# jianhao2016/AllSet

Measured on AMD Instinct MI355X. Metric: edges*d aggregated / sec (V->E->V layer fwd+bwd), higher is better.
Workload: dtype f32

## Files before the change

allset_amd/_lib.py:

```python
from __future__ import annotations

import ctypes
import os
from ctypes import c_char_p, c_float, c_int, c_int64, c_size_t, c_uint64, c_void_p, POINTER

import torch

LIB_PATH = os.path.join(os.path.dirname(os.path.abspath(__file__)), "liballset_hip.so")
ABI_VERSION = 15
CORE_ABI_VERSION = 1

SUM, MEAN, MAX, MIN = 0, 1, 2, 3
F32, BF16 = 0, 1
REDUCE_AS_TREE = 0x100
ARITH_AUTO, ARITH_BF16X6, ARITH_FP16X3 = 0, 1, 2
ACT_NONE, ACT_RELU, ACT_ELU = 0, 1, 2
REDUCE_CODES = {"add": SUM, "sum": SUM, "mean": MEAN, "max": MAX, "min": MIN}

_P = c_void_p
SIGNATURES = {
    "allset_version": [],
    "allset_core_version": [],
    "allset_csr_build_workspace_bytes": [c_int64, c_int64, POINTER(c_size_t)],
    "allset_csr_build": [_P, _P, c_int64, c_int64, c_int64, c_int64, _P, _P, _P, _P, c_size_t, _P],
    "allset_segreduce_fwd": [c_int, c_int, _P, _P, _P, _P, c_int64, _P, c_int64, _P, c_int64, c_int64, c_int64, _P],
    "allset_segreduce_fwd_ex": [c_int, c_int, c_int, c_int64, _P, _P, _P, _P, _P, c_int64, _P, c_int64, _P, c_int64, c_int64,
                                c_int64, _P],
    "allset_segmax_bwd": [_P, _P, _P, _P, _P, _P, c_int64, _P, c_int64, c_int64, c_int64, c_int64, _P],
    "allset_sddmm_rowdot": [c_int, _P, _P, _P, c_int64, _P, c_int64, _P, _P, c_int64, c_int64, c_int64, _P],
    "allset_pma_fwd": [c_int, _P, _P, _P, _P, c_int64, c_float, _P, c_int64, _P, _P, c_int64, c_int64, c_int64, c_int64, _P],
    "allset_pma_fwd_ex": [c_int, c_int, c_int64, _P, _P, _P, _P, _P, c_int64, c_float, _P, c_int64, _P, _P, c_int64, c_int64,
                          c_int64, c_int64, _P],
    "allset_pma_fwd_ld": [c_int, c_int, c_int64, _P, _P, _P, _P, c_int64, _P, c_int64, c_float, _P, c_int64, _P, _P, c_int64,
                          c_int64, c_int64, c_int64, _P],
    "allset_pma_bwd_stats_ld": [c_int, _P, c_int64, _P, c_int64, _P, _P, _P, c_int64, c_int64, c_int64, c_int64, _P],
    "allset_pma_bwd_src_ld": [c_int, c_int, c_int64, _P, _P, _P, _P, _P, c_int64, _P, c_int64, _P, c_int64, c_float, _P, c_int64,
                              _P, c_int64, c_int64, c_int64, c_int64, _P],
    "allset_pma_attention": [_P, _P, _P, _P, _P, c_float, _P, c_int64, c_int64, _P],
    "allset_pma_bwd_stats": [c_int, _P, c_int64, _P, c_int64, _P, _P, _P, c_int64, c_int64, c_int64, _P],
    "allset_pma_bwd_src": [c_int, _P, _P, _P, _P, c_int64, _P, c_int64, _P, c_float, _P, c_int64, _P,
                           c_int64, c_int64, c_int64, c_int64, _P],
    "allset_pma_bwd_src_ex": [c_int, c_int, c_int64, _P, _P, _P, _P, _P, c_int64, _P, c_int64, _P, c_float, _P, c_int64, _P,
                              c_int64, c_int64, c_int64, c_int64, _P],
    "allset_ln_fwd": [_P, c_int64, _P, _P, c_float, c_int, c_float, c_uint64, _P, c_int64, _P, c_int64, c_int64, _P, _P],
    "allset_ln_bwd_partials": [c_int64, c_int64, POINTER(c_int64)],
    "allset_ln_bwd": [_P, c_int64, _P, c_int64, _P, _P, c_int, c_float, c_uint64, _P, c_int64, _P, c_int64,
                      c_int64, c_int64, _P, _P],
# ... 206 lines not shown
    "allset_han_block_relabel": [_P, _P, _P, c_int64, c_int64, _P, _P, _P, _P, _P],
    "allset_han_block_compact_fixed": [_P, _P, _P, _P, _P, _P, _P, _P, c_int64, c_int64, _P, _P, _P, _P, _P],
    "allset_han_block_transpose": [_P, _P, _P, c_int64, c_int64, _P, _P, _P, _P],
    "allset_han_block_compact": [_P, _P, _P, _P, _P, _P, c_int64, c_int64, c_int64, c_int64, _P, _P, _P],
    "allset_han_block_hop_fwd": [c_int64, _P, _P, _P, _P, _P, c_int64, c_float, _P, c_float, c_uint64, _P, _P, c_int64, _P, c_int64, _P,
                                 _P, c_int64, c_int64, c_int64, c_int64, _P],
    "allset_han_block_hop_bwd_stats": [_P, c_int64, _P, _P, c_int64, _P, c_int64, _P, _P, c_float, _P, c_int64, _P, _P, c_int64, c_int64,
                                       c_int64, _P],
    "allset_han_block_hop_bwd_src": [c_int64, _P, _P, _P, _P, _P, _P, c_int64, _P, c_int64, _P, c_float, c_float, c_uint64, _P, _P,
                                     c_int64, _P, c_int64, c_int64, c_int64, c_int64, _P],
    "allset_hattn_supported": [],
    "allset_hattn_coef": [c_int64, _P, _P, _P, _P, _P, _P, c_float, c_float, c_uint64, _P, _P, _P, _P, _P, c_int64, c_int64, c_int64, _P],
    "allset_hattn_hop": [c_int64, _P, _P, _P, _P, _P, _P, _P, c_int64, _P, c_int, c_float, c_uint64, _P, c_int, _P, c_int64, c_int64,
                         c_int64, c_int64, c_int64, _P],
    "allset_hattn_bwd_vertex": [c_int64, _P, _P, _P, _P, _P, _P, _P, _P, c_float, _P, c_int64, _P, c_int64, _P, c_int64, _P, c_int64, _P,
                                _P, _P, c_int64, _P, _P, _P, c_int64, c_int64, c_int64, c_int64, _P],
    "allset_hattn_bwd_edge": [c_int64, _P, _P, _P, c_int64, c_int64, _P],
    "allset_spgemm_bool_bins": [POINTER(c_int64)],
    "allset_spgemm_bool_workspace_bytes": [c_int64, POINTER(c_size_t)],
    "allset_spgemm_bool_count": [_P, _P, _P, _P, c_int64, c_int64, c_int64, _P, _P, c_size_t, _P],
    "allset_spgemm_bool_fill": [_P, _P, _P, _P, c_int64, c_int64, c_int64, _P, c_int64, _P, _P, c_size_t, _P],
    "allset_loo_supported": [c_int64],
    "allset_loo_long_threshold": [],
    "allset_loo_rows": [_P, _P, _P, c_int64, _P, _P, _P, c_int64, _P, c_int64, c_int64, c_int64, c_int64, c_int64, _P],
    "allset_loo_softmax_supported": [c_int64, c_int64],
    "allset_loo_softmax_fwd": [_P, _P, _P, _P, c_int64, c_float, _P, c_int64, _P, _P, c_int64, c_int64, c_int64, c_int64, c_int64,
                               c_int64, _P],
    "allset_loo_softmax_bwd": [_P, _P, _P, _P, c_int64, c_float, _P, c_int64, _P, _P, c_int64, _P, _P, c_int64, _P, _P, _P, c_int64,
                               c_int64, c_int64, c_int64, c_int64, c_int64, _P],
    "allset_scan_rows_supported": [c_int64],
    "allset_scan_rows": [_P, _P, _P, c_int64, _P, _P, c_int64, _P, c_int64, c_int, c_int64, c_int64, c_int64, c_int64, _P],
    "allset_scan_collect": [_P, _P, _P, c_int64, _P, _P, c_int64, _P, _P, c_int, c_float, c_uint64, _P, _P, c_int64, c_int64, c_int64,
                            c_int64, c_int64, _P],
}
EXPORTED_SYMBOLS = sorted(list(SIGNATURES) + ["allset_last_error"])


class AllSetHipError(RuntimeError):
    pass


_lib = None


def load() -> ctypes.CDLL:
    global _lib
    if _lib is not None:
        return _lib
    if not os.path.exists(LIB_PATH):
        raise AllSetHipError(
            f"{LIB_PATH} not found: build it with `python -m allset_amd.build` "
            "(allset_amd has no CPU / eager fallback for the aggregation path)")
    lib = ctypes.CDLL(LIB_PATH)
    for name, argtypes in SIGNATURES.items():
        fn = getattr(lib, name)
        fn.argtypes = argtypes
        fn.restype = c_int
    lib.allset_fused_linear_mask_words.restype = c_int64
    lib.allset_gemm_x6_plane_bytes.restype = c_int64
    lib.allset_gemm_f16x3_plane_bytes.restype = c_int64
    lib.allset_gemm_x6_lnb_partials.restype = c_int64
    lib.allset_input_linear_k.restype = c_int64
    lib.allset_linear_bf16_mask_pitch.restype = c_int64
    lib.allset_sparse_linear_pitch.restype = c_int64
    lib.allset_last_error.argtypes = []
    lib.allset_last_error.restype = c_char_p
# ... 53 lines not shown
```

allset_amd/csrc/segreduce.hip:

```cpp
#include "common.h"
#include "flat_rows.h"
#include "mfma.h"

namespace allset {

enum { kModeSum = 0, kModeExt = 1 };
constexpr int kUnroll = 8;
#ifndef ALLSET_SEG_UNROLL_ONE_SLOT
#define ALLSET_SEG_UNROLL_ONE_SLOT 8
#endif
#ifndef ALLSET_SEG_MAX_LPR
#define ALLSET_SEG_MAX_LPR 64
#endif
constexpr int kBwdUnroll = 4;

template <typename T, int VEC, int LPR, int MODE, bool WEIGHTED>
__global__ __launch_bounds__(kBlock) void segreduce_kernel(
    const int32_t* __restrict__ rowptr, const int32_t* __restrict__ col, const float* __restrict__ w,
    const T* __restrict__ x, int64_t ldx, T* __restrict__ out, int64_t ldo,
    int32_t* __restrict__ argext, int n_t, int d, int mean, float sign, const int32_t* __restrict__ row_order) {
  constexpr int NS = kWave / LPR;
  constexpr int U = NS == 1 ? ALLSET_SEG_UNROLL_ONE_SLOT : kUnroll;
  const unsigned blk = xcd_contiguous_block(blockIdx.x, gridDim.x);
  const int slot_row = static_cast<int>(blk) * kWavesPerBlock + (threadIdx.x >> 6);
// ... 263 lines not shown
  for (int k = 0; k < VEC; ++k) { g.v[k] = 0.f; ap[k] = -1; }
  if (active) {
    g = load_vec<float, VEC>(gout + static_cast<int64_t>(row) * ldg + c0);
    if constexpr (MODE == kModeExt) load_vec_i32<VEC>(argext + static_cast<int64_t>(row) * d + c0, ap);
  }
  for (int base = start; base < end; base += kWave) {
    const int n = min(kWave, end - base);
    const int my_col = lane < n ? col[base + lane] : 0;
    for (int j = 0; j < n; j += NS * kUnroll) {
      Raw<float, VEC> raw[kUnroll];
#pragma unroll
      for (int u = 0; u < kUnroll; ++u) {
        const int jj = j + u * NS + slot;
        const int src = __shfl(my_col, jj & (kWave - 1));
        if (jj < n && active) raw[u] = load_raw<float, VEC>(x + static_cast<int64_t>(src) * ldx + c0);
        else raw[u] = zero_raw<float, VEC>();
      }
      float res = 0.f;
#pragma unroll
      for (int u = 0; u < kUnroll; ++u) {
        const FVec<VEC> v = unpack<float, VEC>(raw[u]);
        float part = 0.f;
#pragma unroll
        for (int k = 0; k < VEC; ++k) {
          if constexpr (MODE == kModeExt) part = (ap[k] == base + j + u * NS + slot) ? fmaf(v.v[k], g.v[k], part) : part;
          else part = fmaf(v.v[k], g.v[k], part);
        }
        part = slot_sum<LPR>(part);
        res = (li == u) ? part : res;
      }
      const int jo = j + li * NS + slot;
      if (li < kUnroll && jo < n) gw[base + jo] = res * scale;
    }
  }
}


template <typename T, int VEC, int LPR>
static void launch_segreduce(int mode_ext, bool weighted, unsigned grid, hipStream_t st,
                             const int32_t* rowptr, const int32_t* col, const float* w, const T* x,
                             int64_t ldx, T* out, int64_t ldo, int32_t* argext, int n_t, int d, int mean,
                             float sign, const int32_t* row_order) {
  if (!mode_ext) {
    if (weighted) segreduce_kernel<T, VEC, LPR, kModeSum, true><<<grid, kBlock, 0, st>>>(rowptr, col, w, x, ldx, out, ldo, argext, n_t, d, mean, sign, row_order);
    else          segreduce_kernel<T, VEC, LPR, kModeSum, false><<<grid, kBlock, 0, st>>>(rowptr, col, w, x, ldx, out, ldo, argext, n_t, d, mean, sign, row_order);
  } else {
    if (weighted) segreduce_kernel<T, VEC, LPR, kModeExt, true><<<grid, kBlock, 0, st>>>(rowptr, col, w, x, ldx, out, ldo, argext, n_t, d, mean, sign, row_order);
    else          segreduce_kernel<T, VEC, LPR, kModeExt, false><<<grid, kBlock, 0, st>>>(rowptr, col, w, x, ldx, out, ldo, argext, n_t, d, mean, sign, row_order);
  }
}

template <typename T, int WIDE>
static void dispatch_flat(bool weighted, hipStream_t st, const int32_t* rowptr, const int32_t* col, const float* w,
                          const T* x, int64_t ldx, T* out, int64_t ldo, int n_t, int d, int mean) {
  with_lpr(pick_lpr(d, WIDE), [&](auto lpr) {
    const unsigned grid = flat_grid<lpr()>(n_t);
    if (weighted) segreduce_flat_kernel<T, WIDE, lpr(), true><<<grid, kBlock, 0, st>>>(rowptr, col, w, x, ldx, out, ldo, n_t, d, mean);
    else          segreduce_flat_kernel<T, WIDE, lpr(), false><<<grid, kBlock, 0, st>>>(rowptr, col, w, x, ldx, out, ldo, n_t, d, mean);
  });
}

template <typename T, int WIDE>
static void dispatch_segreduce(bool wide_ok, int mode_ext, bool weighted, unsigned grid, hipStream_t st,
                               const int32_t* rowptr, const int32_t* col, const float* w, const T* x, int64_t ldx,
                               T* out, int64_t ldo, int32_t* argext, int n_t, int d, int mean, float sign,
                               const int32_t* row_order) {
// ... 102 lines not shown
}

extern "C" int allset_sddmm_rowdot(int reduce, const int32_t* rowptr, const int32_t* col, const float* x,
                                   int64_t ldx, const float* gout, int64_t ldg, const int32_t* argext,
                                   float* gw, int64_t n_t, int64_t n_s, int64_t d, void* stream) {
  clear_error();
  ALLSET_REQUIRE(reduce >= ALLSET_SUM && reduce <= ALLSET_MIN, "sddmm_rowdot: bad reduce %d", reduce);
  ALLSET_REQUIRE(n_t >= 0 && n_s >= 0 && d >= 0, "sddmm_rowdot: negative size");
  ALLSET_REQUIRE(n_t < INT32_MAX && n_s < INT32_MAX && d < INT32_MAX, "sddmm_rowdot: size exceeds int32");
  if (n_t == 0 || n_s == 0) return ALLSET_OK;
  ALLSET_REQUIRE(rowptr && col && x && gout && gw, "sddmm_rowdot: null pointer");
  ALLSET_REQUIRE(ldx >= d && ldg >= d, "sddmm_rowdot: leading dimension smaller than d");
  const bool ext = (reduce == ALLSET_MAX || reduce == ALLSET_MIN);
  ALLSET_REQUIRE(!ext || argext, "sddmm_rowdot: MAX/MIN need argext");
  const hipStream_t st = static_cast<hipStream_t>(stream);
  const unsigned grid = row_grid(n_t);
  const int mean = (reduce == ALLSET_MEAN);
  const int nt = static_cast<int>(n_t), di = static_cast<int>(d);
  const bool vec4 = (d % 4 == 0) && d <= 256 && (ldx % 4 == 0) && (ldg % 4 == 0) && aligned16(x) && aligned16(gout) &&
                    (!ext || aligned16(argext));
  if (vec4) {
    with_lpr(pick_lpr(d), [&](auto lpr) {
      if (ext) sddmm_rowdot_vec_kernel<lpr(), kModeExt><<<grid, kBlock, 0, st>>>(rowptr, col, x, ldx, gout, ldg, argext, gw, nt, di, mean);
      else     sddmm_rowdot_vec_kernel<lpr(), kModeSum><<<grid, kBlock, 0, st>>>(rowptr, col, x, ldx, gout, ldg, nullptr, gw, nt, di, mean);
    });
  } else if (ext) {
    sddmm_rowdot_kernel<kModeExt><<<grid, kBlock, 0, st>>>(rowptr, col, x, ldx, gout, ldg, argext, gw, nt, di, mean);
  } else {
    sddmm_rowdot_kernel<kModeSum><<<grid, kBlock, 0, st>>>(rowptr, col, x, ldx, gout, ldg, nullptr, gw, nt, di, mean);
  }
  ALLSET_LAUNCH_CHECK();
  return ALLSET_OK;
}
```

allset_amd/dist.py:

```python
from __future__ import annotations

import os
from typing import Callable, Optional, Tuple

import torch
import torch.distributed as dist
import torch.nn.functional as F

Tensor = torch.Tensor



def vertex_block(n_v: int, world: int, rank: int) -> Tuple[int, int, int]:
    per = (n_v + world - 1) // world
    return rank * per, (rank + 1) * per, per * world


def partition_hyperedges(sizes: Tensor, world: int, method: str = "contiguous") -> Tensor:
    sizes = sizes.to(torch.int64)
    n_e = sizes.numel()
    if method == "contiguous":
        csum = torch.cumsum(sizes, 0)
        total = int(csum[-1]) if n_e else 0
        mid = csum - sizes // 2
# ... 361 lines not shown
    @staticmethod
    def forward(ctx, part, hg, is_min):
        halo = hg.halo
        r = halo.rank
        v = -part if is_min else part
        key = (_ordered_key(v) << 8) | (255 - r)
        if halo.world == 1 or _skip_collective(halo.group):
            recv = key
        else:
            recv = _all_to_all_rows(key.contiguous(), halo.need_counts, halo.send_counts, halo.group)
        best = torch.full((halo.block, key.shape[1]), -1, dtype=torch.int64, device=key.device)
        if recv.shape[0]:
            best = best.scatter_reduce(0, halo.send_idx.view(-1, 1).expand_as(recv), recv, "amax", include_self=True)
        best_c = best.index_select(0, halo.send_idx)
        if not (halo.world == 1 or _skip_collective(halo.group)):
            best_c = _all_to_all_rows(best_c, halo.send_counts, halo.need_counts, halo.group)
        won = best_c == key
        any_inc = best >= 0
        bits = (best >> 8) & 0xFFFFFFFF
        bits = torch.where(bits >= 0x80000000, bits - 0x80000000, 0xFFFFFFFF - bits)
        val = torch.where(bits >= 0x80000000, bits - 0x100000000, bits).to(torch.int32).view(torch.float32)
        out = torch.where(any_inc, -val if is_min else val, torch.zeros_like(val))
        ctx.save_for_backward(won)
        ctx.halo = halo
        return out

    @staticmethod
    def backward(ctx, gout):
        (won,) = ctx.saved_tensors
        g_c = ctx.halo._gather(gout.contiguous())
        return torch.where(won, g_c, torch.zeros_like(g_c)), None, None


def _hip_deepsets(x, inc, norm, aggr):
    from . import functional as AF
    return AF.deepsets_aggregate(x, inc, norm, aggr)


class HipPmaKernels:

    @staticmethod
    def aggregate(V, alpha, inc, heads, slope):
        from . import functional as AF
        return AF.pma_aggregate(V, alpha, inc, heads, slope)[0]

    @staticmethod
    def fwd(V, alpha, inc, heads, slope):
        from . import ops
        from .functional import _variant, _sizes
        csr = inc.by_dst
        return ops.pma_fwd(csr.rowptr, csr.col, alpha, V, heads, slope, inc.n_dst,
                           variant=_variant(csr, "pma_fwd", inc.n_dst, V, heads), row_order=csr.row_order, sizes=_sizes(csr, V, heads))

    @staticmethod
    def bwd_stats(out, gout, m, l):
        from . import ops
        return ops.pma_bwd_stats(out, gout, m, l)

    @staticmethod
    def merge_pack(o_loc, m_loc, l_loc, m_glob, heads):
        from . import ops
        return ops.pma_merge_pack(o_loc, m_loc, l_loc, m_glob, heads)

    @staticmethod
    def bwd_src(inc, alpha, V, gout, stats, slope):
        from . import ops
        from .functional import _variant, _sizes
        T = inc.by_src
        return ops.pma_bwd_src(T.rowptr, T.col, alpha, V, gout, stats, slope,
                               variant=_variant(T, "pma_bwd_src", V.shape[0], V, alpha.shape[1]), row_order=T.row_order,
                               sizes=_sizes(T, V, alpha.shape[1]))


def _bn_scope(valid_rows: int, group):
    from . import dense
    return dense.sync_bn_rows(valid_rows, group)


def _valid_rows(lo: int, hi: int, n: int) -> int:
    return max(0, min(int(hi), int(n)) - int(lo))


def sharded_deepsets_layer(v2e_conv, e2v_conv, x_owned: Tensor, hg: ShardedHypergraph, aggr: str = "add",
                           dropout: float = 0.0, training: bool = False, group=None,
                           aggregate: Callable = _hip_deepsets, norm: Optional[Tensor] = None,
                           dropout_out: Optional[float] = None) -> Tensor:
    if aggr not in ("add", "sum", "mean", "max", "min"):
        raise ValueError(f"aggr {aggr!r}")
    vv = _valid_rows(hg.v_lo, hg.v_hi, hg.n_v)
    norm = hg.norm if norm is None else norm
    p_out = dropout if dropout_out is None else dropout_out
    use_halo = hg.halo is not None and hg.halo_v2e is not None
    with _bn_scope(vv, group):
        h = v2e_conv._mlp_act(v2e_conv.f_enc, x_owned, v2e_conv.dropout)
    if use_halo:
        e = aggregate(halo_gather(h, hg.halo), hg.halo_v2e, norm, aggr)
    else:
        h_full = all_gather_rows(h, group)
        e = aggregate(h_full, hg.v2e, norm, aggr)
    with _bn_scope(e.shape[0], group):
        e = v2e_conv._mlp_act(v2e_conv.f_dec, e, dropout)
        g = e2v_conv._mlp_act(e2v_conv.f_enc, e, e2v_conv.dropout)
    if aggr in ("max", "min") and use_halo:
        v = _HaloExtremeMerge.apply(aggregate(g, hg.halo_e2v, norm, aggr), hg, aggr == "min")
    elif aggr in ("max", "min"):
        partial = aggregate(g, hg.e2v, norm, aggr)
        v = _ShardedExtremeMerge.apply(partial, hg.local_vertex_has_incidence(), hg, group, aggr == "min")
    elif use_halo:
        v = halo_scatter_add(aggregate(g, hg.halo_e2v, norm, "add"), hg.halo)
    else:
        partial = aggregate(g, hg.e2v, norm, "add")
        v = reduce_scatter_rows(partial, group)
    if aggr == "mean":
        v = v / hg.owned_vertex_degree(group).clamp(min=1).view(-1, 1)
    with _bn_scope(vv, group):
        return e2v_conv._mlp_act(e2v_conv.f_dec, v, p_out)


class _ShardedPmaE2V(torch.autograd.Function):

    @staticmethod
    def forward(ctx, V, alpha, hg, heads, slope, group, K, use_halo=False):
        halo = hg.halo if use_halo else None
        inc = hg.halo_e2v if halo is not None else hg.e2v
        in_dtype = V.dtype
        alpha = alpha.float()
        o_loc, m_loc, l_loc = K.fwd(V, alpha, inc, heads, slope)
        o_loc = o_loc.float()
        n, d = o_loc.shape
        C = d // heads
        has = l_loc > 0
        neg_inf = torch.full_like(m_loc, float("-inf"))
        m_eff = torch.where(has, m_loc, neg_inf)
        if halo is not None:
            m_owned = halo._scatter_max(m_loc.contiguous())
            m_gc = halo.gather_narrow(m_owned)
            if hasattr(K, "merge_pack"):
                packed = K.merge_pack(o_loc, m_loc, l_loc, m_gc, heads)
            else:
                w = l_loc * torch.exp(m_loc - m_gc)
                packed = torch.cat([(o_loc.view(n, heads, C) * w.unsqueeze(-1)).view(n, d), w], dim=1)
            red = halo.scatter_add_narrow(packed)
            numer, l_g = red[:, :d], red[:, d:].contiguous()
            inv = torch.where(l_g > 0, 1.0 / (l_g + 1e-16), torch.zeros_like(l_g))
# ... 725 lines not shown
```

allset_amd/functional.py:

```python
from __future__ import annotations

from typing import Optional, Tuple

import torch
from torch.autograd.function import once_differentiable

from . import _lib, ops
from ._lib import MAX, MEAN, MIN, REDUCE_CODES, SUM
from .incidence import Incidence, LeaveOneOutIncidence

Tensor = torch.Tensor


def _variant(csr, kind: str, n_rows: int, x: Tensor, heads: int = 1) -> int:
    es = x.element_size()
    wide = 16 // es
    d = x.shape[1]
    ok = (d % wide == 0 and d <= 64 * wide and x.stride(0) % wide == 0 and x.data_ptr() % 16 == 0
          and (d // max(heads, 1)) % wide == 0)
    if not ok:
        return 1
    if d * es <= 128 and csr.max_deg <= 512:
        return 2
    return csr.variant(kind, n_rows)
# ... 24 lines not shown
def _check_rows(x: Tensor, inc: Incidence) -> None:
    if not (inc.src_extent <= x.shape[0] <= inc.n_src):
        raise ValueError(f"source matrix has {x.shape[0]} rows; incidence needs between {inc.src_extent} "
                         f"and {inc.n_src}")


class _RouteWeights(torch.autograd.Function):

    @staticmethod
    def forward(ctx, w, perm, inv_perm):
        ctx.save_for_backward(inv_perm)
        return w.index_select(0, perm)

    @staticmethod
    @once_differentiable
    def backward(ctx, g):
        (inv_perm,) = ctx.saved_tensors
        return g.index_select(0, inv_perm), None, None


def _routed(norm: Tensor, inc: Incidence, dst: bool) -> Tensor:
    csr = inc.by_dst if dst else inc.by_src
    perm, inv = (inc.perm_dst_long(), inc.inv_perm_dst()) if dst else (inc.perm_src_long(), inc.inv_perm_src())
    if norm.grad_fn is None:
        return _RouteWeights.apply(norm.reshape(-1).to(torch.float32), perm, inv)
    cache = norm.__dict__.setdefault("_allset_routed", {})
    key = (id(csr), norm._version, torch.is_grad_enabled())
    hit = cache.get(key)
    if hit is None:
        hit = cache[key] = _RouteWeights.apply(norm.reshape(-1).to(torch.float32), perm, inv)
    return hit


class _SegReduce(torch.autograd.Function):
    @staticmethod
    def forward(ctx, x: Tensor, w_dst: Optional[Tensor], w_src: Optional[Tensor], inc: Incidence, reduce: int):
        csr = inc.by_dst
        ext = reduce in (MAX, MIN)
        out, arg = ops.segreduce(reduce, csr.rowptr, csr.col, w_dst, x, inc.n_dst, want_arg=ext,
                                 variant=1 if ext else _variant(csr, "segreduce", inc.n_dst, x), row_order=csr.row_order,
                                 split=_split(csr, x))
        need_gw = w_dst is not None and ctx.needs_input_grad[1]
        ctx.inc, ctx.reduce, ctx.n_s, ctx.need_gw = inc, reduce, x.shape[0], need_gw
        ctx.save_for_backward(x if need_gw else None, w_dst, w_src, arg)
        return out

    @staticmethod
    @once_differentiable
    def backward(ctx, gout: Tensor):
        x, w_dst, w_src, arg = ctx.saved_tensors
        inc, reduce = ctx.inc, ctx.reduce
        T = inc.by_src
        gx = gw = None
        gout = gout.contiguous()
        if reduce in (MAX, MIN) or ctx.need_gw:
            if gout.dtype != torch.float32:
                raise _lib.AllSetHipError("max/min backward and weight gradients are fp32-only; bf16 storage covers "
                                          "sum/mean and the PMA path")
        if ctx.needs_input_grad[0]:
            if w_dst is not None and w_src is None:
                w_src = w_dst[inc.pos_dst_of_src().long()]
            if reduce in (SUM, MEAN):
                if reduce == MEAN:
                    inv = inc.inv_count_by_src()
                    w_src = inv if w_src is None else w_src * inv
                gx, _ = ops.segreduce(SUM, T.rowptr, T.col, w_src, gout, ctx.n_s,
                                      variant=_variant(T, "segreduce", ctx.n_s, gout), row_order=T.row_order,
                                      split=_split(T, gout) if ctx.n_s == T.n_rows else -1)
            else:
                gx = ops.segmax_bwd(T.rowptr, T.col, inc.pos_dst_of_src(), w_src, arg, gout, ctx.n_s)
        if ctx.need_gw:
            csr = inc.by_dst
            gw = ops.sddmm_rowdot(reduce, csr.rowptr, csr.col, x, gout, arg)
        return gx, gw, None, None, None


def deepsets_aggregate(x: Tensor, inc: Incidence, norm: Optional[Tensor] = None, aggr: str = "add") -> Tensor:
    if aggr not in REDUCE_CODES:
        raise ValueError(f"unknown aggr {aggr!r}")
    _lib.require_device(x)
    _check_rows(x, inc)
    if norm is not None and norm.requires_grad:
        w_dst = _routed(norm, inc, True)
        w_src = _routed(norm, inc, False).detach()
    else:
        w_dst, w_src = inc.weights(norm)
    return _SegReduce.apply(x, w_dst, w_src, inc, REDUCE_CODES[aggr])


def _loo_expand(x: Tensor, loo: LeaveOneOutIncidence, s_src: Optional[Tensor], s_seg: Optional[Tensor]) -> Tensor:
    return ops.loo_rows(loo.e_rowptr, loo.e_col, x, s_src, s_seg, long_seg=loo.long_seg if loo.n_long else None, n_long=loo.n_long)


def _loo_collect(y: Tensor, loo: LeaveOneOutIncidence, s_seg: Optional[Tensor], w_inc: Optional[Tensor], n_rows: int) -> Tensor:
    t = ops.loo_rows(loo.e_rowptr, None, y, None, s_seg, long_seg=loo.long_seg if loo.n_long else None, n_long=loo.n_long)
    out, _ = ops.segreduce(SUM, loo.v_rowptr, loo.v_col, w_inc, t, n_rows)
    return out


class _LooV2E(torch.autograd.Function):
    @staticmethod
    def forward(ctx, x: Tensor, loo: LeaveOneOutIncidence, f):
        ctx.loo, ctx.f, ctx.n_rows = loo, f, x.shape[0]
        return _loo_expand(x, loo, f.v2e_src, f.v2e_seg)

    @staticmethod
    @once_differentiable
    def backward(ctx, gout: Tensor):
        f = ctx.f
        return _loo_collect(gout.contiguous(), ctx.loo, f.v2e_seg, f.v2e_src_inc, ctx.n_rows), None, None


class _LooE2V(torch.autograd.Function):
    @staticmethod
    def forward(ctx, y: Tensor, loo: LeaveOneOutIncidence, f):
        ctx.loo, ctx.f = loo, f
        return _loo_collect(y, loo, f.e2v_seg, f.e2v_row_inc, loo.n_dst)

    @staticmethod
    @once_differentiable
# ... 912 lines not shown
```

allset_amd/layers.py:

```python
from __future__ import annotations

import math
from typing import Tuple, Optional, Union

import os

import torch
import torch.nn as nn
import torch.nn.functional as F

from . import dense
from . import functional as AF
from .incidence import Incidence, LooDirection, cached_incidence

Tensor = torch.Tensor
EdgeIndex = Union[Tensor, Incidence]


def glorot(tensor: Optional[Tensor]) -> None:
    if tensor is not None:
        bound = math.sqrt(6.0 / (tensor.size(-2) + tensor.size(-1)))
        with torch.no_grad():
            tensor.uniform_(-bound, bound)

# ... 432 lines not shown
    def __repr__(self):
        return '{}({}, {}, heads={})'.format(self.__class__.__name__, self.in_channels, self.out_channels, self.heads)


class HalfNLHconv(nn.Module):

    def __init__(self, in_dim, hid_dim, out_dim, num_layers, dropout, Normalization='bn', InputNorm=False,
                 heads=1, attention=True):
        super().__init__()
        self.attention = attention
        self.dropout = dropout
        if self.attention:
            self.prop = PMA(in_dim, hid_dim, out_dim, num_layers, heads=heads)
        elif num_layers > 0:
            self.f_enc = MLP(in_dim, hid_dim, hid_dim, num_layers, dropout, Normalization, InputNorm)
            self.f_dec = MLP(hid_dim, hid_dim, out_dim, num_layers, dropout, Normalization, InputNorm)
        else:
            self.f_enc = nn.Identity()
            self.f_dec = nn.Identity()

    def reset_parameters(self):
        if self.attention:
            self.prop.reset_parameters()
        else:
            for f in (self.f_enc, self.f_dec):
                if not isinstance(f, nn.Identity):
                    f.reset_parameters()

    def takes_pre_dropout(self, x: Tensor) -> bool:
        if self.attention:
            return self.prop.takes_pre_dropout(x)
        return isinstance(self.f_enc, MLP) and self.f_enc.takes_pre_dropout(x)

    def forward(self, x, edge_index: EdgeIndex, norm, aggr='add', _post_dropout: Optional[float] = None, _pre_dropout: float = 0.0):
        post = _post_dropout is not None
        if _pre_dropout and not (self.takes_pre_dropout(x) and (aggr is not None or self.attention)):
            raise ValueError("HalfNLHconv.forward(_pre_dropout=...) needs takes_pre_dropout(x)")
        if isinstance(edge_index, LooDirection):
            if self.attention:
                if not edge_index.attention:
                    raise NotImplementedError("exclude-self data without the expansion reaches the PMA conv (attention=True, "
                                              "AllSetTransformer) only when asked for: preprocessing.exclude_self(data, normtype, "
                                              "attention=True) takes the leave-one-out softmax; or expand the edge list with "
                                              "preprocessing.expand_edge_index instead")
                if norm is not None and norm.requires_grad:
                    raise NotImplementedError("exclude-self data without the expansion takes no per-incidence weight (LearnMask is a "
                                              "parameter per EXPANDED incidence); expand the edge list with "
                                              "preprocessing.expand_edge_index instead")
                if post and self.training:
                    return self.prop.forward_exclude_self(x, edge_index, _post=float(_post_dropout), _pre=float(_pre_dropout))
                x = self.prop.forward_exclude_self(x, edge_index, _pre=float(_pre_dropout))
                return relu_dropout(x, _post_dropout, self.training) if post else x
            if norm is not None and norm.requires_grad:
                raise NotImplementedError("exclude-self data without the expansion takes no per-incidence weight (LearnMask is a parameter "
                                          "per EXPANDED incidence); expand the edge list with preprocessing.expand_edge_index instead")
            if aggr is None:
                raise ValueError("aggr was not passed!")
            x = self._mlp_act(self.f_enc, x, self.dropout, pre=_pre_dropout)
            x = AF.deepsets_aggregate_exclude_self(x, edge_index.loo, edge_index.direction, aggr, edge_index.normtype)
            return self._mlp_act(self.f_dec, x, _post_dropout if post else 0.0)
        if self.attention:
            if post and self.training:
                return self.prop(x, edge_index, _post=float(_post_dropout), _pre=float(_pre_dropout))
            x = self.prop(x, edge_index, _pre=float(_pre_dropout))
            return relu_dropout(x, _post_dropout, self.training) if post else x
        if aggr is None:
            raise ValueError("aggr was not passed!")
        x = self._mlp_act(self.f_enc, x, self.dropout, pre=_pre_dropout)
        inc = _as_incidence(edge_index, x.shape[0])
        x = AF.deepsets_aggregate(x, inc, norm, aggr)
        return self._mlp_act(self.f_dec, x, _post_dropout if post else 0.0)

    def _mlp_act(self, mlp, x, p, in_cb: int = 0, out_cb: int = 0, pre: float = 0.0):
        if isinstance(mlp, MLP):
            return mlp(x, _post=p, _in_cb=in_cb, _out_cb=out_cb, _pre=pre)
        return relu_dropout(mlp(x), p, self.training)
```

allset_amd/ops.py:

```python
from __future__ import annotations

from collections import defaultdict
from ctypes import byref, c_int64 as c_int64_t, c_size_t, c_void_p
from typing import Dict, List, NamedTuple, Optional, Sequence, Tuple

import torch

from . import _lib
from ._lib import check, ptr, require_device, stream_of, on_device

Tensor = torch.Tensor


class KernelTimer:

    def __init__(self):
        self.events: Dict[str, List[Tuple[torch.cuda.Event, torch.cuda.Event, int]]] = defaultdict(list)

    def summary(self) -> Dict[str, Dict[str, float]]:
        out = {}
        for name, evs in self.events.items():
            ms = [s.elapsed_time(e) for s, e, _ in evs]
            out[name] = dict(calls=len(ms), total_ms=sum(ms), avg_ms=sum(ms) / len(ms),
                             algo_bytes=sum(b for _, _, b in evs) / len(evs))
# ... 185 lines not shown
    return order.to(torch.int32).contiguous()


def segreduce(reduce: int, rowptr: Tensor, col: Tensor, w: Optional[Tensor], x: Tensor, n_t: int,
              want_arg: bool = False, variant: int = 0, row_order: Optional[Tensor] = None, split: int = -1
              ) -> Tuple[Tensor, Optional[Tensor]]:
    dev = require_device(rowptr, col, w, x)
    code = _dtype_code(x, "segreduce")
    es = x.element_size()
    x = _rowmajor(x)
    n_s, d = x.shape
    out = torch.empty((n_t, d), dtype=x.dtype, device=dev)
    arg = torch.empty((n_t, d), dtype=torch.int32, device=dev) if want_arg else None
    if w is not None:
        _f32(w, "segreduce weights")
        w = w.contiguous()
    nnz = col.numel()
    algo = nnz * (es * d + 4 + (4 if w is not None else 0)) + (n_t + 1) * 4 + n_t * d * es
    with on_device(dev), _timed("segreduce_fwd", dev, algo):
        if row_order is not None and row_order.numel() != n_t:
            row_order = None
        lib = _lib.load()
        if 0 < split < n_t and not want_arg and rowptr.numel() == n_t + 1:
            check(lib.allset_segreduce_fwd_ex(reduce, code, 1, nnz, None, ptr(rowptr), ptr(col), ptr(w), ptr(x), _ld(x),
                                              ptr(out), max(d, 1), None, split, n_s, d, stream_of(dev)), "allset_segreduce_fwd_ex")
            check(lib.allset_segreduce_fwd_ex(reduce, code, 2, nnz, None, ptr(rowptr[split:]), ptr(col), ptr(w), ptr(x), _ld(x),
                                              ptr(out[split:]), max(d, 1), None, n_t - split, n_s, d, stream_of(dev)),
                  "allset_segreduce_fwd_ex")
        else:
            check(lib.allset_segreduce_fwd_ex(reduce, code, variant, nnz, ptr(row_order), ptr(rowptr), ptr(col), ptr(w), ptr(x), _ld(x),
                                              ptr(out), max(d, 1), ptr(arg), n_t, n_s, d, stream_of(dev)),
                  "allset_segreduce_fwd_ex")
    return out, arg


def segmax_bwd(rowptrT: Tensor, colT: Tensor, posT: Tensor, wT: Optional[Tensor], argext: Tensor, gout: Tensor,
               n_s: int) -> Tensor:
    dev = require_device(rowptrT, colT, posT, wT, argext, gout)
    _f32(gout, "segmax_bwd")
    gout = _rowmajor(gout)
    n_t, d = gout.shape
    if colT.numel() == 0:
        return torch.zeros((n_s, d), dtype=gout.dtype, device=dev)
    gx = torch.empty((n_s, d), dtype=gout.dtype, device=dev)
    algo = colT.numel() * (4 * d + 4 * d + 8) + (n_s + 1) * 4 + n_s * d * 4
    with on_device(dev), _timed("segmax_bwd", dev, algo):
        check(_lib.load().allset_segmax_bwd(ptr(rowptrT), ptr(colT), ptr(posT), ptr(wT), ptr(argext), ptr(gout),
                                            _ld(gout), ptr(gx), max(d, 1), n_s, n_t, d, stream_of(dev)),
              "allset_segmax_bwd")
    return gx


def sddmm_rowdot(reduce: int, rowptr: Tensor, col: Tensor, x: Tensor, gout: Tensor, argext: Optional[Tensor]) -> Tensor:
    dev = require_device(rowptr, col, x, gout, argext)
    _f32(x, "sddmm_rowdot")
    x, gout = _rowmajor(x), _rowmajor(gout)
    n_s, d = x.shape
    n_t = gout.shape[0]
    gw = torch.empty(col.numel(), dtype=torch.float32, device=dev)
    if col.numel() == 0:
        return gw
    algo = col.numel() * (4 * d + 8) + (n_t + 1) * 4 + n_t * d * 4
    with on_device(dev), _timed("sddmm_rowdot", dev, algo):
        check(_lib.load().allset_sddmm_rowdot(reduce, ptr(rowptr), ptr(col), ptr(x), _ld(x), ptr(gout), _ld(gout),
                                              ptr(argext), ptr(gw), n_t, n_s, d, stream_of(dev)),
              "allset_sddmm_rowdot")
# ... 1309 lines not shown
```

include/allset_hip_ext.h:

```cpp
#ifndef ALLSET_HIP_EXT_H
#define ALLSET_HIP_EXT_H

#include "allset_hip.h"

#ifdef __cplusplus
extern "C" {
#endif

#define ALLSET_ABI_VERSION 15


int allset_ln_fwd(const float* x, int64_t ldx, const float* gamma, const float* beta, float eps, int relu_in,
                  float p, uint64_t seed, float* y, int64_t ldy, float* stats, int64_t n, int64_t d,
                  const uint64_t* seed_base, void* stream);

int allset_ln_bwd_partials(int64_t n, int64_t d, int64_t* n_partials);
int allset_ln_bwd(const float* gy, int64_t ldg, const float* x, int64_t ldx, const float* stats, const float* gamma,
                  int relu_in, float p, uint64_t seed, float* gx, int64_t ldgx, float* partials, int64_t n_partials,
                  int64_t n, int64_t d, const uint64_t* seed_base, void* stream);

int allset_relu_dropout_fwd(const float* x, float p, uint64_t seed, float* y, int64_t numel,
                            const uint64_t* seed_base, void* stream);
int allset_relu_dropout_bwd(const float* gy, const float* y, float p, float* gx, int64_t numel, void* stream);

// ... 453 lines not shown
int allset_hattn_bwd_edge(int64_t nnz, const int32_t* rowptr, const float* ge_e, float* gae, int64_t n_e, int64_t H, void* stream);

int allset_spgemm_bool_bins(int64_t* bins );
int allset_spgemm_bool_workspace_bytes(int64_t n_a, size_t* bytes);
int allset_spgemm_bool_count(const int32_t* rowptrA, const int32_t* colA, const int32_t* rowptrB, const int32_t* colB, int64_t n_a,
                             int64_t n_b, int64_t n_c, int32_t* cnt, void* workspace, size_t workspace_bytes, void* stream);
int allset_spgemm_bool_fill(const int32_t* rowptrA, const int32_t* colA, const int32_t* rowptrB, const int32_t* colB, int64_t n_a,
                            int64_t n_b, int64_t n_c, const int32_t* rowptrC, int64_t nnz_c, int32_t* colC, const void* workspace,
                            size_t workspace_bytes, void* stream);

int allset_loo_supported(int64_t d);
int allset_loo_long_threshold(void);
int allset_loo_rows(const int32_t* rowptr, const int32_t* col, const float* src, int64_t lds, const float* s_src, const float* s_seg,
                    float* out, int64_t ldo, const int32_t* long_seg, int64_t n_long, int64_t n_seg, int64_t n_src, int64_t nnz,
                    int64_t d, void* stream);

int allset_loo_softmax_supported(int64_t d, int64_t heads);
int allset_loo_softmax_fwd(const int32_t* rowptr, const int32_t* col, const float* alpha, const float* V, int64_t ldv, float slope,
                           float* out, int64_t ldo, float* lse, const int32_t* long_seg, int64_t n_long, int64_t n_seg,
                           int64_t n_src, int64_t nnz, int64_t d, int64_t heads, void* stream);
int allset_loo_softmax_bwd(const int32_t* rowptr, const int32_t* col, const float* alpha, const float* V, int64_t ldv, float slope,
                           const float* out, int64_t ldo, const float* lse, const float* gout, int64_t ldg, const float* glse,
                           float* gV, int64_t ldgv, float* galpha, float* scratch, const int32_t* long_seg, int64_t n_long,
                           int64_t n_seg, int64_t n_src, int64_t nnz, int64_t d, int64_t heads, void* stream);

int allset_scan_rows_supported(int64_t d);
int allset_scan_rows(const int32_t* rowptr, const int32_t* col, const float* src, int64_t lds, const float* s_src, float* out,
                     int64_t ldo, const int32_t* long_seg, int64_t n_long, int reverse, int64_t n_seg, int64_t n_src, int64_t nnz,
                     int64_t d, void* stream);
int allset_scan_collect(const int32_t* rowptr, const int32_t* col, const float* t, int64_t ldt, const float* r_self, const float* x,
                        int64_t ldx, const float* s, const float* bias, int act, float p, uint64_t seed, const uint64_t* seed_base,
                        float* y, int64_t ldy, int64_t n_t, int64_t n_pos, int64_t d, int64_t width, void* stream);

#ifdef __cplusplus
}
#endif
#endif
```

Baseline: 229.6 billion.

## Gather sparsity-packed rows in segment-sum forward when encoder output is mostly zero

Adds a pack kernel that compresses each 128-wide f32 row into a 64-dword record holding a 128-bit nonzero mask plus up to 60 nonzero values. A new segment-sum kernel gathers these half-size records, expands them in LDS with popcount indexing, and falls back to the dense row when a row overflows the cap. The packed path is used in training when the conv's dropout is at least 0.5, on the premise that ReLU plus dropout leaves rows mostly zero, so gather traffic per incidence drops. In exchange it adds an extra pack pass over the rows, LDS expansion work, and divergent fallback loads for dense rows.

```diff
diff --git a/allset_amd/_lib.py b/allset_amd/_lib.py
--- a/allset_amd/_lib.py
+++ b/allset_amd/_lib.py
@@ -13,6 +13,7 @@
 SUM, MEAN, MAX, MIN = 0, 1, 2, 3
 F32, BF16 = 0, 1
 REDUCE_AS_TREE = 0x100
+PACK_PITCH_DW, PACK_CAP = 64, 60
 ARITH_AUTO, ARITH_BF16X6, ARITH_FP16X3 = 0, 1, 2
 ACT_NONE, ACT_RELU, ACT_ELU = 0, 1, 2
 REDUCE_CODES = {"add": SUM, "sum": SUM, "mean": MEAN, "max": MAX, "min": MIN}
@@ -285,6 +286,8 @@
     "allset_scan_rows": [_P, _P, _P, c_int64, _P, _P, c_int64, _P, c_int64, c_int, c_int64, c_int64, c_int64, c_int64, _P],
     "allset_scan_collect": [_P, _P, _P, c_int64, _P, _P, c_int64, _P, _P, c_int, c_float, c_uint64, _P, _P, c_int64, c_int64, c_int64,
                             c_int64, c_int64, _P],
+    "allset_pack_rows_f32": [_P, c_int64, _P, c_int64, c_int64, _P],
+    "allset_segreduce_packed_fwd": [c_int, _P, _P, _P, _P, _P, c_int64, _P, c_int64, c_int64, c_int64, c_int64, _P],
 }
 EXPORTED_SYMBOLS = sorted(list(SIGNATURES) + ["allset_last_error"])
 
diff --git a/allset_amd/csrc/segreduce.hip b/allset_amd/csrc/segreduce.hip
--- a/allset_amd/csrc/segreduce.hip
+++ b/allset_amd/csrc/segreduce.hip
@@ -319,6 +319,158 @@
       const int jo = j + li * NS + slot;
       if (li < kUnroll && jo < n) gw[base + jo] = res * scale;
     }
+  }
+}
+
+constexpr int kPackRowsPerWave = 4;
+constexpr int kExpand = 2;
+
+__device__ __forceinline__ void lds_wave_handoff() {
+  __builtin_amdgcn_fence(__ATOMIC_SEQ_CST, "wavefront");
+  __builtin_amdgcn_wave_barrier();
+}
+
+__device__ __forceinline__ uint32_t all_ones_if_bit(uint32_t m, int b) {
+  return static_cast<uint32_t>(__builtin_amdgcn_sbfe(static_cast<int>(m), static_cast<unsigned>(b), 1u));
+}
+
+__device__ __forceinline__ int mask_count(const uint4& m) { return __popc(m.x) + __popc(m.y) + __popc(m.z) + __popc(m.w); }
+
+__global__ __launch_bounds__(kBlock) void pack_rows_kernel(const float* __restrict__ x, int64_t ldx, uint32_t* __restrict__ packed, int64_t n) {
+  __shared__ __attribute__((aligned(16))) uint32_t image[kWavesPerBlock][kPackRowsPerWave][kPackPitchDw];
+  const int wave = threadIdx.x >> 6, lane = lane_id();
+  const int slot = lane >> 5, li = lane & 31;
+  const int64_t row0 = (static_cast<int64_t>(blockIdx.x) * kWavesPerBlock + wave) * kPackRowsPerWave;
+  if (row0 >= n) return;
+  uint4 raw[kPackRowsPerWave / 2];
+#pragma unroll
+  for (int p = 0; p < kPackRowsPerWave / 2; ++p) {
+    const int64_t r = row0 + 2 * p + slot;
+    raw[p] = r < n ? *reinterpret_cast<const uint4*>(x + r * ldx + 4 * li) : make_uint4(0u, 0u, 0u, 0u);
+  }
+#pragma unroll
+  for (int p = 0; p < kPackRowsPerWave / 2; ++p) {
+    uint32_t* dst = image[wave][2 * p + slot];
+    const uint32_t v[4] = {raw[p].x, raw[p].y, raw[p].z, raw[p].w};
+    const unsigned nib = (v[0] != 0u ? 1u : 0u) | (v[1] != 0u ? 2u : 0u) | (v[2] != 0u ? 4u : 0u) | (v[3] != 0u ? 8u : 0u);
+    const int g = li >> 3, sh = 4 * (li & 7);
+    unsigned mw = nib << sh;
+    mw |= __shfl_xor(mw, 1);
+    mw |= __shfl_xor(mw, 2);
+    mw |= __shfl_xor(mw, 4);
+    uint4 m;
+    m.x = __shfl(mw, slot * 32);
+    m.y = __shfl(mw, slot * 32 + 8);
+    m.z = __shfl(mw, slot * 32 + 16);
+    m.w = __shfl(mw, slot * 32 + 24);
+    int pos = 4 + (g > 0 ? __popc(m.x) : 0) + (g > 1 ? __popc(m.y) : 0) + (g > 2 ? __popc(m.z) : 0) + __popc(mw & ((1u << sh) - 1u));
+#pragma unroll
+    for (int i = 0; i < 4; ++i) {
+      if ((nib >> i) & 1u) {
+        if (pos < kPackPitchDw) dst[pos] = v[i];
+        ++pos;
+      }
+    }
+    if (li == 0) *reinterpret_cast<uint4*>(dst) = m;
+  }
+  lds_wave_handoff();
+  const int rr = lane >> 4, q = 4 * (lane & 15);
+  const uint32_t* src = image[wave][rr];
+  const int k = mask_count(*reinterpret_cast<const uint4*>(src));
+  uint4 o = *reinterpret_cast<const uint4*>(src + q);
+  if (q + 0 >= 4 + k) o.x = 0u;
+  if (q + 1 >= 4 + k) o.y = 0u;
+  if (q + 2 >= 4 + k) o.z = 0u;
+  if (q + 3 >= 4 + k) o.w = 0u;
+  if (row0 + rr < n) *reinterpret_cast<uint4*>(packed + (row0 + rr) * kPackPitchDw + q) = o;
+}
+
+constexpr int kImagePad = 128;
+__global__ __launch_bounds__(kBlock) __attribute__((amdgpu_waves_per_eu(8, 8))) void segreduce_packed_kernel(
+    const int32_t* __restrict__ rowptr, const int32_t* __restrict__ col, const uint32_t* __restrict__ packed,
+    const float* __restrict__ x, int64_t ldx, float* __restrict__ out, int64_t ldo, int n_t, int mean,
+    const int32_t* __restrict__ row_order) {
+  constexpr int VEC = 4, LPR = 32, NS = 2, U = kUnroll;
+  __shared__ __attribute__((aligned(16))) uint32_t image[kWavesPerBlock * U * NS * kPackPitchDw + kImagePad];
+  const unsigned blk = xcd_contiguous_block(blockIdx.x, gridDim.x);
+  const int slot_row = static_cast<int>(blk) * kWavesPerBlock + (threadIdx.x >> 6);
+  if (slot_row >= n_t) return;
+  const int row = row_order ? row_order[slot_row] : slot_row;
+  const int wave = threadIdx.x >> 6, lane = lane_id();
+  const int slot = lane / LPR, li = lane % LPR;
+  const int start = rowptr[row], end = rowptr[row + 1];
+  const uint32_t below = (1u << li) - 1u;
+  uint32_t* const mine = image + (wave * U * NS + slot) * kPackPitchDw;
+  float acc[VEC];
+#pragma unroll
+  for (int g = 0; g < VEC; ++g) acc[g] = 0.f;
+
+  for (int base = start; base < end; base += kWave) {
+    const int n = min(kWave, end - base);
+    int my_col = 0;
+    if (lane < n) my_col = col[base + lane];
+    for (int j = 0; j < n; j += NS * U) {
+      uint2 raw[U];
+#pragma unroll
+      for (int u = 0; u < U; ++u) {
+        const int jj = j + u * NS + slot;
+        const int src = __shfl(my_col, jj & (kWave - 1));
+        if (jj < n) raw[u] = *reinterpret_cast<const uint2*>(packed + static_cast<int64_t>(src) * kPackPitchDw + 2 * li);
+        else raw[u] = make_uint2(0u, 0u);
+      }
+#pragma unroll
+      for (int u = 0; u < U; ++u) *reinterpret_cast<uint2*>(mine + u * NS * kPackPitchDw + 2 * li) = raw[u];
+      lds_wave_handoff();
+#pragma unroll
+      for (int u0 = 0; u0 < U; u0 += kExpand) {
+        if (j + u0 * NS >= n) break;
+        uint4 m[kExpand];
+#pragma unroll
+        for (int e = 0; e < kExpand; ++e) m[e] = *reinterpret_cast<const uint4*>(mine + (u0 + e) * NS * kPackPitchDw);
+        uint32_t v[kExpand][VEC];
+        bool over[kExpand];
+        bool any_over = false;
+#pragma unroll
+        for (int e = 0; e < kExpand; ++e) {
+          const uint32_t* r = mine + (u0 + e) * NS * kPackPitchDw;
+          const int c1 = 4 + __popc(m[e].x), c2 = c1 + __popc(m[e].y), c3 = c2 + __popc(m[e].z);
+          over[e] = c3 + __popc(m[e].w) > 4 + kPackCap;
+          any_over |= over[e];
+          v[e][0] = r[4 + __popc(m[e].x & below)] & all_ones_if_bit(m[e].x, li);
+          v[e][1] = r[c1 + __popc(m[e].y & below)] & all_ones_if_bit(m[e].y, li);
+          v[e][2] = r[c2 + __popc(m[e].z & below)] & all_ones_if_bit(m[e].z, li);
+          v[e][3] = r[c3 + __popc(m[e].w & below)] & all_ones_if_bit(m[e].w, li);
+        }
+        if (__any(any_over)) {
+#pragma unroll
+          for (int e = 0; e < kExpand; ++e) {
+            const int src = __shfl(my_col, (j + (u0 + e) * NS + slot) & (kWave - 1));
+            if (over[e]) {
+              const uint32_t* xr = reinterpret_cast<const uint32_t*>(x + static_cast<int64_t>(src) * ldx) + li;
+#pragma unroll
+              for (int g = 0; g < VEC; ++g) v[e][g] = xr[32 * g];
+            }
+          }
+        }
+#pragma unroll
+        for (int e = 0; e < kExpand; ++e)
+#pragma unroll
+          for (int g = 0; g < VEC; ++g) acc[g] = fmaf(1.f, __uint_as_float(v[e][g]), acc[g]);
+      }
+      lds_wave_handoff();
+    }
+  }
+
+#pragma unroll
+  for (int off = LPR; off < kWave; off <<= 1)
+#pragma unroll
+    for (int g = 0; g < VEC; ++g) acc[g] += __shfl_xor(acc[g], off);
+
+  if (slot == 0) {
+    const float scale = mean ? 1.f / static_cast<float>(max(end - start, 1)) : 1.f;
+    float* o = out + static_cast<int64_t>(row) * ldo + li;
+#pragma unroll
+    for (int g = 0; g < VEC; ++g) o[32 * g] = acc[g] * scale;
   }
 }
 
@@ -487,3 +639,47 @@
   ALLSET_LAUNCH_CHECK();
   return ALLSET_OK;
 }
+
+static inline bool aligned256(const void* p) { return (reinterpret_cast<uintptr_t>(p) & 255u) == 0; }
+
+extern "C" int allset_pack_rows_f32(const float* x, int64_t ldx, void* packed, int64_t n, int64_t d, void* stream) {
+  clear_error();
+  ALLSET_REQUIRE(n >= 0 && d >= 0, "pack_rows_f32: negative size");
+  ALLSET_REQUIRE(n < INT32_MAX, "pack_rows_f32: size exceeds int32");
+  if (d != 128) {
+    set_error("pack_rows_f32: built for d = 128 only (got %lld)", static_cast<long long>(d));
+    return ALLSET_ERR_UNSUPPORTED;
+  }
+  if (n == 0) return ALLSET_OK;
+  ALLSET_REQUIRE(x && packed, "pack_rows_f32: null x/packed");
+  ALLSET_REQUIRE(ldx >= d && ldx % 4 == 0 && aligned16(x), "pack_rows_f32: rows of x must be 16-byte aligned (pointer and leading dimension)");
+  ALLSET_REQUIRE(aligned256(packed), "pack_rows_f32: the packed buffer must be 256-byte aligned");
+  const int64_t rows_per_block = static_cast<int64_t>(kWavesPerBlock) * kPackRowsPerWave;
+  const unsigned grid = static_cast<unsigned>((n + rows_per_block - 1) / rows_per_block);
+  pack_rows_kernel<<<grid, kBlock, 0, static_cast<hipStream_t>(stream)>>>(x, ldx, static_cast<uint32_t*>(packed), n);
+  ALLSET_LAUNCH_CHECK();
+  return ALLSET_OK;
+}
+
+extern "C" int allset_segreduce_packed_fwd(int reduce, const int32_t* row_order, const int32_t* rowptr, const int32_t* col,
+                                           const void* packed, const float* x, int64_t ldx, float* out, int64_t ldo, int64_t n_t,
+                                           int64_t n_s, int64_t d, void* stream) {
+  clear_error();
+  ALLSET_REQUIRE(reduce == ALLSET_SUM || reduce == ALLSET_MEAN, "segreduce_packed_fwd: reduce must be SUM or MEAN (got %d)", reduce);
+  ALLSET_REQUIRE(n_t >= 0 && n_s >= 0 && d >= 0, "segreduce_packed_fwd: negative size");
+  ALLSET_REQUIRE(n_t < INT32_MAX && n_s < INT32_MAX, "segreduce_packed_fwd: size exceeds int32");
+  if (d != 128) {
+    set_error("segreduce_packed_fwd: built for d = 128 only (got %lld)", static_cast<long long>(d));
+    return ALLSET_ERR_UNSUPPORTED;
+  }
+  if (n_t == 0) return ALLSET_OK;
+  ALLSET_REQUIRE(rowptr && out, "segreduce_packed_fwd: null rowptr/out");
+  ALLSET_REQUIRE(n_s == 0 || (col && packed && x), "segreduce_packed_fwd: null col/packed/x with n_s > 0");
+  ALLSET_REQUIRE(ldx >= d && ldo >= d && ldx % 4 == 0 && ldo % 4 == 0 && aligned16(x) && aligned16(out),
+                 "segreduce_packed_fwd: rows of x and out must be 16-byte aligned (pointers and leading dimensions)");
+  ALLSET_REQUIRE(aligned256(packed), "segreduce_packed_fwd: the packed buffer must be 256-byte aligned");
+  segreduce_packed_kernel<<<row_grid(n_t), kBlock, 0, static_cast<hipStream_t>(stream)>>>(
+      rowptr, col, static_cast<const uint32_t*>(packed), x, ldx, out, ldo, static_cast<int>(n_t), reduce == ALLSET_MEAN, row_order);
+  ALLSET_LAUNCH_CHECK();
+  return ALLSET_OK;
+}
diff --git a/allset_amd/dist.py b/allset_amd/dist.py
--- a/allset_amd/dist.py
+++ b/allset_amd/dist.py
@@ -417,9 +417,15 @@
         return torch.where(won, g_c, torch.zeros_like(g_c)), None, None
 
 
-def _hip_deepsets(x, inc, norm, aggr):
+def _hip_deepsets(x, inc, norm, aggr, packed_rows=False):
     from . import functional as AF
-    return AF.deepsets_aggregate(x, inc, norm, aggr)
+    return AF.deepsets_aggregate(x, inc, norm, aggr, packed_rows=packed_rows)
+
+
+def _forward_aggregate(aggregate: Callable, conv) -> Callable:
+    if aggregate is _hip_deepsets and conv.mostly_zero_enc():
+        return lambda x, inc, norm, aggr: _hip_deepsets(x, inc, norm, aggr, packed_rows=True)
+    return aggregate
 
 
 class HipPmaKernels:
@@ -476,25 +482,26 @@
     norm = hg.norm if norm is None else norm
     p_out = dropout if dropout_out is None else dropout_out
     use_halo = hg.halo is not None and hg.halo_v2e is not None
+    agg_v2e, agg_e2v = _forward_aggregate(aggregate, v2e_conv), _forward_aggregate(aggregate, e2v_conv)
     with _bn_scope(vv, group):
         h = v2e_conv._mlp_act(v2e_conv.f_enc, x_owned, v2e_conv.dropout)
     if use_halo:
-        e = aggregate(halo_gather(h, hg.halo), hg.halo_v2e, norm, aggr)
+        e = agg_v2e(halo_gather(h, hg.halo), hg.halo_v2e, norm, aggr)
     else:
         h_full = all_gather_rows(h, group)
-        e = aggregate(h_full, hg.v2e, norm, aggr)
+        e = agg_v2e(h_full, hg.v2e, norm, aggr)
     with _bn_scope(e.shape[0], group):
         e = v2e_conv._mlp_act(v2e_conv.f_dec, e, dropout)
         g = e2v_conv._mlp_act(e2v_conv.f_enc, e, e2v_conv.dropout)
     if aggr in ("max", "min") and use_halo:
-        v = _HaloExtremeMerge.apply(aggregate(g, hg.halo_e2v, norm, aggr), hg, aggr == "min")
+        v = _HaloExtremeMerge.apply(agg_e2v(g, hg.halo_e2v, norm, aggr), hg, aggr == "min")
     elif aggr in ("max", "min"):
-        partial = aggregate(g, hg.e2v, norm, aggr)
+        partial = agg_e2v(g, hg.e2v, norm, aggr)
         v = _ShardedExtremeMerge.apply(partial, hg.local_vertex_has_incidence(), hg, group, aggr == "min")
     elif use_halo:
-        v = halo_scatter_add(aggregate(g, hg.halo_e2v, norm, "add"), hg.halo)
+        v = halo_scatter_add(agg_e2v(g, hg.halo_e2v, norm, "add"), hg.halo)
     else:
-        partial = aggregate(g, hg.e2v, norm, "add")
+        partial = agg_e2v(g, hg.e2v, norm, "add")
         v = reduce_scatter_rows(partial, group)
     if aggr == "mean":
         v = v / hg.owned_vertex_degree(group).clamp(min=1).view(-1, 1)
diff --git a/allset_amd/functional.py b/allset_amd/functional.py
--- a/allset_amd/functional.py
+++ b/allset_amd/functional.py
@@ -80,14 +80,38 @@
     return hit
 
 
+_PACKED_GATHER = True
+
+
+def set_packed_gather(on: bool) -> None:
+    global _PACKED_GATHER
+    _PACKED_GATHER = bool(on)
+
+
+def packed_gather() -> bool:
+    return _PACKED_GATHER
+
+
+def _takes_packed(x: Tensor, w_dst: Optional[Tensor], inc: Incidence, reduce: int) -> bool:
+    if not (_PACKED_GATHER and x.dtype == torch.float32 and x.dim() == 2 and x.shape[1] == 128 and x.is_contiguous()
+            and x.data_ptr() % 16 == 0 and reduce in (SUM, MEAN) and w_dst is None and x.shape[0] > 0 and inc.n_dst > 0):
+        return False
+    csr = inc.by_dst
+    return _variant(csr, "segreduce", inc.n_dst, x) == 1 and not (0 < _split(csr, x) < inc.n_dst)
+
+
 class _SegReduce(torch.autograd.Function):
     @staticmethod
-    def forward(ctx, x: Tensor, w_dst: Optional[Tensor], w_src: Optional[Tensor], inc: Incidence, reduce: int):
+    def forward(ctx, x: Tensor, w_dst: Optional[Tensor], w_src: Optional[Tensor], inc: Incidence, reduce: int, packed_rows: bool = False):
         csr = inc.by_dst
         ext = reduce in (MAX, MIN)
-        out, arg = ops.segreduce(reduce, csr.rowptr, csr.col, w_dst, x, inc.n_dst, want_arg=ext,
-                                 variant=1 if ext else _variant(csr, "segreduce", inc.n_dst, x), row_order=csr.row_order,
-                                 split=_split(csr, x))
+        if packed_rows and _takes_packed(x, w_dst, inc, reduce):
+            out = ops.segreduce_packed(reduce, csr.rowptr, csr.col, ops.pack_rows(x), x, inc.n_dst, row_order=csr.row_order)
+            arg = None
+        else:
+            out, arg = ops.segreduce(reduce, csr.rowptr, csr.col, w_dst, x, inc.n_dst, want_arg=ext,
+                                     variant=1 if ext else _variant(csr, "segreduce", inc.n_dst, x), row_order=csr.row_order,
+                                     split=_split(csr, x))
         need_gw = w_dst is not None and ctx.needs_input_grad[1]
         ctx.inc, ctx.reduce, ctx.n_s, ctx.need_gw = inc, reduce, x.shape[0], need_gw
         ctx.save_for_backward(x if need_gw else None, w_dst, w_src, arg)
@@ -120,10 +144,11 @@
         if ctx.need_gw:
             csr = inc.by_dst
             gw = ops.sddmm_rowdot(reduce, csr.rowptr, csr.col, x, gout, arg)
-        return gx, gw, None, None, None
-
-
-def deepsets_aggregate(x: Tensor, inc: Incidence, norm: Optional[Tensor] = None, aggr: str = "add") -> Tensor:
+        return gx, gw, None, None, None, None
+
+
+def deepsets_aggregate(x: Tensor, inc: Incidence, norm: Optional[Tensor] = None, aggr: str = "add",
+                       packed_rows: bool = False) -> Tensor:
     if aggr not in REDUCE_CODES:
         raise ValueError(f"unknown aggr {aggr!r}")
     _lib.require_device(x)
@@ -133,7 +158,7 @@
         w_src = _routed(norm, inc, False).detach()
     else:
         w_dst, w_src = inc.weights(norm)
-    return _SegReduce.apply(x, w_dst, w_src, inc, REDUCE_CODES[aggr])
+    return _SegReduce.apply(x, w_dst, w_src, inc, REDUCE_CODES[aggr], bool(packed_rows))
 
 
 def _loo_expand(x: Tensor, loo: LeaveOneOutIncidence, s_src: Optional[Tensor], s_seg: Optional[Tensor]) -> Tensor:
diff --git a/allset_amd/layers.py b/allset_amd/layers.py
--- a/allset_amd/layers.py
+++ b/allset_amd/layers.py
@@ -488,6 +488,9 @@
             return self.prop.takes_pre_dropout(x)
         return isinstance(self.f_enc, MLP) and self.f_enc.takes_pre_dropout(x)
 
+    def mostly_zero_enc(self) -> bool:
+        return bool(self.training and not self.attention and self.dropout >= 0.5)
+
     def forward(self, x, edge_index: EdgeIndex, norm, aggr='add', _post_dropout: Optional[float] = None, _pre_dropout: float = 0.0):
         post = _post_dropout is not None
         if _pre_dropout and not (self.takes_pre_dropout(x) and (aggr is not None or self.attention)):
@@ -524,7 +527,7 @@
             raise ValueError("aggr was not passed!")
         x = self._mlp_act(self.f_enc, x, self.dropout, pre=_pre_dropout)
         inc = _as_incidence(edge_index, x.shape[0])
-        x = AF.deepsets_aggregate(x, inc, norm, aggr)
+        x = AF.deepsets_aggregate(x, inc, norm, aggr, packed_rows=self.mostly_zero_enc())
         return self._mlp_act(self.f_dec, x, _post_dropout if post else 0.0)
 
     def _mlp_act(self, mlp, x, p, in_cb: int = 0, out_cb: int = 0, pre: float = 0.0):
diff --git a/allset_amd/ops.py b/allset_amd/ops.py
--- a/allset_amd/ops.py
+++ b/allset_amd/ops.py
@@ -241,6 +241,37 @@
                                               ptr(out), max(d, 1), ptr(arg), n_t, n_s, d, stream_of(dev)),
                   "allset_segreduce_fwd_ex")
     return out, arg
+
+
+def pack_rows(x: Tensor) -> Tensor:
+    dev = require_device(x)
+    _f32(x, "pack_rows")
+    x = _rowmajor(x)
+    n, d = x.shape
+    packed = torch.empty((n, _lib.PACK_PITCH_DW), dtype=torch.int32, device=dev)
+    with on_device(dev), _timed("pack_rows", dev, n * (4 * d + 4 * _lib.PACK_PITCH_DW)):
+        check(_lib.load().allset_pack_rows_f32(ptr(x), _ld(x), ptr(packed), n, d, stream_of(dev)), "allset_pack_rows_f32")
+    return packed
+
+
+def segreduce_packed(reduce: int, rowptr: Tensor, col: Tensor, packed: Tensor, x: Tensor, n_t: int,
+                     row_order: Optional[Tensor] = None) -> Tensor:
+    dev = require_device(rowptr, col, packed, x)
+    _f32(x, "segreduce_packed")
+    x = _rowmajor(x)
+    n_s, d = x.shape
+    if packed.dtype != torch.int32 or tuple(packed.shape) != (n_s, _lib.PACK_PITCH_DW) or not packed.is_contiguous():
+        raise _lib.AllSetHipError(f"segreduce_packed: packed must be contiguous int32[{n_s}, {_lib.PACK_PITCH_DW}] (ops.pack_rows)")
+    out = torch.empty((n_t, d), dtype=x.dtype, device=dev)
+    nnz = col.numel()
+    algo = nnz * (4 * _lib.PACK_PITCH_DW + 4) + (n_t + 1) * 4 + n_t * d * 4
+    with on_device(dev), _timed("segreduce_fwd", dev, algo):
+        if row_order is not None and row_order.numel() != n_t:
+            row_order = None
+        check(_lib.load().allset_segreduce_packed_fwd(reduce, ptr(row_order), ptr(rowptr), ptr(col), ptr(packed), ptr(x), _ld(x),
+                                                      ptr(out), max(d, 1), n_t, n_s, d, stream_of(dev)),
+              "allset_segreduce_packed_fwd")
+    return out
 
 
 def segmax_bwd(rowptrT: Tensor, colT: Tensor, posT: Tensor, wT: Optional[Tensor], argext: Tensor, gout: Tensor,
diff --git a/include/allset_hip_ext.h b/include/allset_hip_ext.h
--- a/include/allset_hip_ext.h
+++ b/include/allset_hip_ext.h
@@ -509,6 +509,11 @@
                         int64_t ldx, const float* s, const float* bias, int act, float p, uint64_t seed, const uint64_t* seed_base,
                         float* y, int64_t ldy, int64_t n_t, int64_t n_pos, int64_t d, int64_t width, void* stream);
 
+enum { kPackPitchDw = 64, kPackCap = 60 };
+int allset_pack_rows_f32(const float* x, int64_t ldx, void* packed, int64_t n, int64_t d, void* stream);
+int allset_segreduce_packed_fwd(int reduce, const int32_t* row_order, const int32_t* rowptr, const int32_t* col, const void* packed,
+                                const float* x, int64_t ldx, float* out, int64_t ldo, int64_t n_t, int64_t n_s, int64_t d, void* stream);
+
 #ifdef __cplusplus
 }
 #endif
```

After: 244.1 billion (median of 6 runs). 1.06x the previous value.
